# ginevracoal/robustBNNs

Measured on AMD Instinct MI355X. Metric: attack-samples/sec (test_pts x posterior_samples x PGD_iters), higher is better.
Workload: dtype f32 (full-width operands as three f16 pieces: 6 exact f16 MFMA product terms per fp32 product, f32 accumulate)

## Files before the change

robustbnns_amd/csrc/rbnn_triple.hip:

```cpp
#include "rbnn_pieces.hpp"
#include <algorithm>
#include <cstdlib>

namespace {

#ifndef RBNN_X3_PAIR_NOP
#define RBNN_X3_PAIR_NOP 0
#endif
#if RBNN_X3_PAIR_NOP
#define RBNN_X3_PAIR_PAD "\n\ts_nop 1"
#else
#define RBNN_X3_PAIR_PAD ""
#endif
#define RBNN_X3_PAIR_BODY \
    "v_bfe_i32 %[me], %[mw], %[b0], 1\n\t" \
    "v_bfe_i32 %[mo], %[mw], %[b1], 1\n\t" \
    "v_bfi_b32 %[me], %[me], %[cp], %[cn]\n\t" \
    "v_bfi_b32 %[mo], %[mo], %[cp], %[cn]\n\t" \
    "v_fma_mixlo_f16 %[d0], %[ge], %[me], 0\n\t" \
    "v_fma_mixhi_f16 %[d0], %[go], %[mo], 0\n\t" \
    "v_fma_mix_f32 %[re], %[ge], %[me], -%[d0] op_sel_hi:[0,0,1]\n\t" \
    "v_fma_mix_f32 %[ro], %[go], %[mo], -%[d0] op_sel:[0,0,1] op_sel_hi:[0,0,1]\n\t" \
    "v_cvt_pk_f16_f32 %[d1], %[re], %[ro]\n\t" \
    "v_fma_mixlo_f16 %[d2], -%[d1], %[one], %[re] op_sel_hi:[1,0,0]\n\t" \
    "v_fma_mixhi_f16 %[d2], -%[d1], %[one], %[ro] op_sel:[1,0,0] op_sel_hi:[1,0,0]" RBNN_X3_PAIR_PAD
#define RBNN_X3_PAIR_OPS \
    : [d0] "=&v"(d0), [d1] "=&v"(d1), [d2] "=&v"(d2), [me] "=&v"(me), [mo] "=&v"(mo), [re] "=&v"(re), [ro] "=&v"(ro) \
    : [ge] "v"(ge), [go] "v"(go), [mw] "v"(mw), [cp] "v"(cp), [cn] "v"(cn), [one] "v"(one), [b0] "n"(BIT), [b1] "n"(BIT + 1)
template <int BIT, bool FIRST>
__device__ __forceinline__ void split3_pair(float ge, float go, unsigned mw, unsigned cp, unsigned cn, float one,
                                            unsigned& d0, unsigned& d1, unsigned& d2) {
    unsigned me, mo;
    float re, ro;
    if constexpr (FIRST) asm volatile("s_nop 7\n\t" RBNN_X3_PAIR_BODY RBNN_X3_PAIR_OPS);
    else asm volatile(RBNN_X3_PAIR_BODY RBNN_X3_PAIR_OPS);
}

template <bool FIRST>
__device__ __forceinline__ void split3_pair_m(float ge, float go, float me, float mo, float one, unsigned& d0, unsigned& d1, unsigned& d2) {
    float re, ro;
#define RBNN_X3_PAIRM_BODY \
    "v_fma_mixlo_f16 %[d0], %[ge], %[me], 0\n\t" \
    "v_fma_mixhi_f16 %[d0], %[go], %[mo], 0\n\t" \
    "v_fma_mix_f32 %[re], %[ge], %[me], -%[d0] op_sel_hi:[0,0,1]\n\t" \
    "v_fma_mix_f32 %[ro], %[go], %[mo], -%[d0] op_sel:[0,0,1] op_sel_hi:[0,0,1]\n\t" \
    "v_cvt_pk_f16_f32 %[d1], %[re], %[ro]\n\t" \
    "v_fma_mixlo_f16 %[d2], -%[d1], %[one], %[re] op_sel_hi:[1,0,0]\n\t" \
    "v_fma_mixhi_f16 %[d2], -%[d1], %[one], %[ro] op_sel:[1,0,0] op_sel_hi:[1,0,0]" RBNN_X3_PAIR_PAD
#define RBNN_X3_PAIRM_OPS \
    : [d0] "=&v"(d0), [d1] "=&v"(d1), [d2] "=&v"(d2), [re] "=&v"(re), [ro] "=&v"(ro) \
    : [ge] "v"(ge), [go] "v"(go), [me] "v"(me), [mo] "v"(mo), [one] "v"(one)
    if constexpr (FIRST) asm volatile("s_nop 7\n\t" RBNN_X3_PAIRM_BODY RBNN_X3_PAIRM_OPS);
    else asm volatile(RBNN_X3_PAIRM_BODY RBNN_X3_PAIRM_OPS);
}


__global__ void triple_rows_kernel(const float* __restrict__ src, long long rows, int cols, int ld_src, float scale,
                                   const rbnn_dev_scale* __restrict__ ds, uint4* __restrict__ dst, int groups, int grouped) {
    const long long i = (long long)blockIdx.x * blockDim.x + threadIdx.x;
    if (i >= rows * groups) return;
    if (ds) scale = ds->scale;
    const long long r = i / groups;
    const int g = (int)(i % groups);
    const float* const p = src + r * ld_src + 8 * g;
    union { f16x8 v; uint4 u; } o[3];
#pragma unroll
    for (int j = 0; j < 8; ++j) {
        const float v = (8 * g + j < cols) ? p[j] * scale : 0.f;
        _Float16 q[3];
        pieces_of<3>(v, q);
        o[0].v[j] = q[0]; o[1].v[j] = q[1]; o[2].v[j] = q[2];
    }
    if (grouped) {
        uint4* const out = dst + (((r >> 4) * (groups >> 2) + (g >> 2)) * 192 + (r & 15) * 4 + (g & 3));
        out[0] = o[0].u; out[64] = o[1].u; out[128] = o[2].u;
        return;
    }
    uint4* const out = dst + (r * (groups >> 2) + (g >> 2)) * 12 + (g & 3);
    out[0] = o[0].u; out[4] = o[1].u; out[8] = o[2].u;
}

struct FwdX3Args {
    const char* X;  int ldx;  int N;
    const char* W;  long long w_sample_bytes;  int ldw;  int KT;
    const float* b;  const float* W2;  const float* b2;  int C;  int H;
    const int* sidx;  int S;  int NT;  float out_scale;
    float* P;  uint32_t* mask;  float* dact;  int out_kind;
    const rbnn_dev_scale* x_ds;
    long long x_sample_bytes;  char* hid;  float hid_scale;  const rbnn_dev_scale* hid_ds;
    unsigned x_group_bytes, x_stage_bytes;
};

template <int ACT, int WH, int HTW, int WN, int NTW, bool LAYER2, bool XF32 = false>
__global__ void __launch_bounds__(64 * WH * WN, WH * WN / 4) fc_forward_x3_kernel(const FwdX3Args a) {
    constexpr int BH = WH * HTW * 16, BN = WN * NTW * 16;
    constexpr int PLANEB = (BH + BN) * 64;
    constexpr int TILEB = 3 * PLANEB;
    constexpr bool BITMASK = (ACT == RBNN_ACT_RELU || ACT == RBNN_ACT_LEAKY);
    constexpr int NW = WH * WN;
    constexpr int WPP = BH / 16 / NW, XPP = BN / 16 / NW;
    static_assert((BH / 16) % NW == 0 && (BN / 16) % NW == 0, "whole pieces per wave");
    static_assert(HTW % 2 == 0 && HTW <= 8, "a wave's h range is whole 32-bit mask words, at most 4");
    static_assert(WH * BN * 64 <= 2 * TILEB, "the Z^T reduction scratch aliases the tile buffers");
    extern __shared__ __attribute__((aligned(16))) float lds[];
    char* const ldsb = (char*)lds;
    float* const zred = lds;

    int id;
    if (!item_of_block(blockIdx.x, a.NT * a.S, id)) return;
    constexpr int SB = 4;
    int ntile, s;
    {
        const int full = a.S / SB, per = SB * a.NT;
        if (id < full * per) { ntile = (id % per) / SB; s = (id / per) * SB + id % SB; }
        else { const int rem = id - full * per, cnt = a.S - full * SB; ntile = rem / cnt; s = full * SB + rem % cnt; }
    }
    const int tid = threadIdx.x, lane = tid & 63, li = lane & 15, lg = lane >> 4;
    const int wave = __builtin_amdgcn_readfirstlane(tid >> 6);
    const int wave_h = wave % WH, wave_n = wave / WH;
    const int sw = a.sidx ? a.sidx[s] : s;
    const float out_scale = a.x_ds ? a.out_scale * a.x_ds->inv_scale : a.out_scale;
    const float hid_scale = (!LAYER2 && a.hid_ds) ? a.hid_ds->scale : a.hid_scale;
    const char* const Ws = a.W + (long long)sw * a.w_sample_bytes;
    const char* const Xs = a.X + (long long)s * a.x_sample_bytes;
    const int n0 = ntile * BN;
    const int HW = a.H >> 5;
    const int prow = lane >> 2;
    const unsigned src_off = (unsigned)(prow * 64 + ((lane & 3) ^ swz(prow)) * 16);
    const int foff = li * 64 + ((lg ^ swz(li)) * 16);
    auto sw8 = [](int r) { return ((r >> 1) & 1) | (((r >> 2) & 1) << 2); };
    const unsigned src_off_f = (unsigned)((lane >> 3) * 128 + (((lane & 7) ^ sw8(lane >> 3)) * 16));
    const int foff_f0 = li * 128 + (((2 * lg) ^ sw8(li)) * 16), foff_f1 = li * 128 + (((2 * lg + 1) ^ sw8(li)) * 16);

    f32x4 zacc[NTW];
#pragma unroll
    for (int nt = 0; nt < NTW; ++nt) zacc[nt] = (f32x4){0.f, 0.f, 0.f, 0.f};
    if (NW == 8 && wave >= 4) __builtin_amdgcn_s_setprio(1);

    unsigned xrow[XPP], wrow[WPP];
#pragma unroll
    for (int i = 0; i < XPP; ++i) xrow[i] = (unsigned)min((n0 >> 4) + wave + NW * i, ((a.N + 15) >> 4) - 1) * a.x_group_bytes + (XF32 ? src_off_f : src_off);
#pragma unroll
    for (int i = 0; i < WPP; ++i) wrow[i] = (unsigned)(wave + NW * i) * (unsigned)a.KT * 3072u + src_off;

    constexpr int PPS = WPP + XPP;
    const int G = (a.H / BH) * a.KT;
    auto piece = [&](int c, int kt, int buf, int j) {
        char* const T = ldsb + buf * TILEB;
        const char* src;
        char* dst;
        if (j < WPP) {
            src = Ws + (long long)c * BH * a.ldw * 6 + (wrow[j < WPP ? j : 0] + (unsigned)kt * 3072u);
            dst = T + (wave + NW * j) * 3072;
        } else {
            src = Xs + (xrow[j >= WPP ? j - WPP : 0] + (unsigned)kt * a.x_stage_bytes);
            dst = T + (BH / 16 + wave + NW * (j - WPP)) * 3072;
        }
        const auto gsrc = (const __attribute__((address_space(1))) void*)src;
        const auto ldst = (__attribute__((address_space(3))) void*)(uintptr_t)(uint32_t)(uintptr_t)dst;
        __builtin_amdgcn_global_load_lds(gsrc, ldst, 16, 0, 0);
        __builtin_amdgcn_global_load_lds(gsrc, ldst, 16, 1024, 0);
        if (!(XF32 && j >= WPP)) __builtin_amdgcn_global_load_lds(gsrc, ldst, 16, 2048, 0);
    };
#pragma unroll
    for (int i = 0; i < PPS; ++i) piece(0, 0, 0, i);
    ring_wait_barrier<0>();

    f32x4 acc[HTW][NTW];
#pragma unroll
    for (int ht = 0; ht < HTW; ++ht)
#pragma unroll
        for (int nt = 0; nt < NTW; ++nt) acc[ht][nt] = (f32x4){0.f, 0.f, 0.f, 0.f};

    int kt = 0, ch = 0;
    for (int g = 0; g < G; ++g) {
        const int buf = g & 1;
        const bool wrap = kt + 1 == a.KT, last = g + 1 == G;
        const int ktn = last ? kt : (wrap ? 0 : kt + 1), chn = (wrap && !last) ? ch + 1 : ch;
        const char* const Wt = ldsb + buf * TILEB + (wave_h * HTW) * 3072 + foff;
        const char* const Xt = ldsb + buf * TILEB + (BH / 16 + wave_n * NTW) * 3072 + foff;
        f16x8 b0[NTW], b1[NTW], b2[NTW], a0, a1, a2, a0n, a1n, a2n;
        if (!(RBNN_ABL & 1)) {
#pragma unroll
            for (int i = 0; i < PPS; ++i) piece(chn, ktn, buf ^ 1, i);
        }
        if constexpr (XF32) {
            const char* const Xf = ldsb + buf * TILEB + (BH / 16 + wave_n * NTW) * 3072;
            f32x4 x0[NTW], x1[NTW];
#pragma unroll
            for (int nt = 0; nt < NTW; ++nt) {
                x0[nt] = *(const f32x4*)(Xf + nt * 3072 + foff_f0);
                x1[nt] = *(const f32x4*)(Xf + nt * 3072 + foff_f1);
            }
#pragma unroll
            for (int nt = 0; nt < NTW; ++nt) {
                union { f16x8 v; unsigned w[4]; } q0, q1, q2;
                split3_plain_pair(x0[nt][0], x0[nt][1], 1.f, q0.w[0], q1.w[0], q2.w[0]);
                split3_plain_pair(x0[nt][2], x0[nt][3], 1.f, q0.w[1], q1.w[1], q2.w[1]);
                split3_plain_pair(x1[nt][0], x1[nt][1], 1.f, q0.w[2], q1.w[2], q2.w[2]);
                split3_plain_pair(x1[nt][2], x1[nt][3], 1.f, q0.w[3], q1.w[3], q2.w[3]);
                b0[nt] = q0.v; b1[nt] = q1.v; b2[nt] = q2.v;
            }
        } else {
#pragma unroll
            for (int nt = 0; nt < NTW; ++nt) {
                b0[nt] = *(const f16x8*)(Xt + nt * 3072);
                b1[nt] = *(const f16x8*)(Xt + nt * 3072 + 1024);
                b2[nt] = *(const f16x8*)(Xt + nt * 3072 + 2048);
            }
        }
        a0 = *(const f16x8*)(Wt);
        a1 = *(const f16x8*)(Wt + 1024);
        a2 = *(const f16x8*)(Wt + 2048);
        a0n = a0; a1n = a1; a2n = a2;
#pragma unroll
        for (int ht = 0; ht < HTW; ++ht) {
#pragma unroll
            for (int k = 0; k < 6; ++k) {
                const f16x8 av = (k == 1) ? a2 : ((k == 2 || k == 3) ? a1 : a0);
#pragma unroll
                for (int nt = 0; nt < NTW; ++nt) {
                    const f16x8 bv = (k == 0) ? b2[nt] : ((k == 2 || k == 4) ? b1[nt] : b0[nt]);
                    acc[ht][nt] = MFMA_H(av, bv, acc[ht][nt]);
                }
                if (k == 0 && ht + 1 < HTW) {
                    a0n = *(const f16x8*)(Wt + (ht + 1) * 3072);
                    a1n = *(const f16x8*)(Wt + (ht + 1) * 3072 + 1024);
                    a2n = *(const f16x8*)(Wt + (ht + 1) * 3072 + 2048);
                }
            }
            a0 = a0n; a1 = a1n; a2 = a2n;
        }
        {
            __builtin_amdgcn_sched_group_barrier(0x100, 3 * NTW + 3, 0);
#pragma unroll
            for (int ht = 0; ht < HTW; ++ht) {
                __builtin_amdgcn_sched_group_barrier(0x008, 3 * NTW, 0);
                if (ht + 1 < HTW) __builtin_amdgcn_sched_group_barrier(0x100, 3, 0);
                __builtin_amdgcn_sched_group_barrier(0x008, 3 * NTW, 0);
            }
        }
        if (!(RBNN_ABL & 2)) ring_wait_barrier<0>();
        const int hc0 = ch * BH;
        kt = wrap ? 0 : kt + 1;
        ch = wrap ? ch + 1 : ch;
        if (!wrap) continue;

        if (RBNN_ABL & 8) {
            float t = 0.f;
#pragma unroll
            for (int ht = 0; ht < HTW; ++ht)
#pragma unroll
                for (int nt = 0; nt < NTW; ++nt) { t += acc[ht][nt][0] + acc[ht][nt][1] + acc[ht][nt][2] + acc[ht][nt][3]; acc[ht][nt] = (f32x4){0.f, 0.f, 0.f, 0.f}; }
            if (t == 12345.678f) a.P[tid] = t;
            continue;
        }
        const int hw0 = hc0 + (wave_h * HTW) * 16;
        unsigned mine[NTW];
#pragma unroll
        for (int nt = 0; nt < NTW; ++nt) mine[nt] = 0u;
#pragma unroll
        for (int ht = 0; ht < HTW; ++ht) {
            const int hrow = hw0 + ht * 16 + 4 * lg;
            const f32x4 bias = *(const f32x4*)(a.b + (long long)sw * a.H + hrow);
            f32x4 w2f = (f32x4){0.f, 0.f, 0.f, 0.f};
            if (LAYER2 && li < a.C) w2f = *(const f32x4*)(a.W2 + ((long long)sw * a.C + li) * a.H + hrow);
#pragma unroll
            for (int nt = 0; nt < NTW; ++nt) {
                const int n = n0 + (wave_n * NTW + nt) * 16 + li;
                f32x4 v = acc[ht][nt] * out_scale + bias, hv;
                acc[ht][nt] = (f32x4){0.f, 0.f, 0.f, 0.f};
                unsigned bits = 0;
#pragma unroll
                for (int r = 0; r < 4; ++r) {
                    bits |= (v[r] > 0.f ? 1u : 0u) << r;
                    hv[r] = act_fwd<ACT>(v[r]);
                }
                if (BITMASK) {
                    unsigned part = bits << (16 * (ht & 1) + 4 * lg);
                    part |= __shfl_xor(part, 16);
                    part |= __shfl_xor(part, 32);
                    if (lg == (ht >> 1)) mine[nt] |= part;
                }
                if (!BITMASK && a.dact && n < a.N) {
                    f32x4 dv;
#pragma unroll
                    for (int r = 0; r < 4; ++r) dv[r] = act_grad_from_value<ACT>(hv[r]);
                    *(f32x4*)(a.dact + ((long long)s * a.N + n) * a.H + hrow) = dv;
                }
                if (LAYER2) {
#pragma unroll
                    for (int r = 0; r < 4; ++r) zacc[nt] = MFMA16(w2f[r], hv[r], zacc[nt]);
                } else {
#ifdef RBNN_X3_L1_ABL_NOSTORE
                    if (n < a.N && hv[0] == 1.2345e-30f) {
#else
                    if (n < a.N) {
#endif
                        const long long blk = ((long long)s * HW + (hrow >> 5)) * ((a.N + 15) >> 4) + (n >> 4);
#ifdef RBNN_X3_L1_ABL_SMALL
                        char* const row = a.hid + ((blk * 2048) & 0xFFC00) + (n & 15) * 128 + ((hrow >> 4) & 1) * 64 + lg * 16;
#else
                        char* const row = a.hid + blk * 2048 + (n & 15) * 128 + ((hrow >> 4) & 1) * 64 + lg * 16;
#endif
                        *(f32x4*)row = hv * hid_scale;
                    }
                }
            }
        }
        if (BITMASK && a.mask) {
#pragma unroll
            for (int nt = 0; nt < NTW; ++nt) {
                const int n = n0 + (wave_n * NTW + nt) * 16 + li;
                if (lg < HTW / 2 && n < a.N) a.mask[((long long)s * HW + (hw0 >> 5) + lg) * mask_ld(a.N) + n] = mine[nt];
            }
        }
    }
    if (RBNN_ABL & 2) ring_wait_barrier<0>();

    if (!LAYER2) return;
#pragma unroll
    for (int nt = 0; nt < NTW; ++nt)
        *(f32x4*)(zred + (wave_h * BN + (wave_n * NTW + nt) * 16 + li) * 16 + 4 * lg) = zacc[nt];
    __syncthreads();
    if (tid < BN) {
        const int n = n0 + tid;
        float z[16];
#pragma unroll
        for (int q = 0; q < 4; ++q) {
            f32x4 sum = *(const f32x4*)(zred + tid * 16 + 4 * q);
#pragma unroll
            for (int w = 1; w < WH; ++w) sum += *(const f32x4*)(zred + (w * BN + tid) * 16 + 4 * q);
#pragma unroll
            for (int r = 0; r < 4; ++r) z[4 * q + r] = sum[r];
        }
        float m = -INFINITY;
#pragma unroll
        for (int c = 0; c < 16; ++c) {
            if (c < a.C) { z[c] += a.b2[(long long)sw * a.C + c]; m = fmaxf(m, z[c]); }
            else z[c] = 0.f;
        }
        if (a.out_kind == RBNN_OUT_PROBS) {
            float den = 0.f;
#pragma unroll
            for (int c = 0; c < 16; ++c) if (c < a.C) { z[c] = expf(z[c] - m); den += z[c]; }
#pragma unroll
            for (int c = 0; c < 16; ++c) if (c < a.C) z[c] = z[c] / den;
        }
        if (n < a.N) {
            float* const dst = a.P + ((long long)s * a.N + n) * RBNN_CPAD;
#pragma unroll
            for (int q = 0; q < 4; ++q) *(f32x4*)(dst + 4 * q) = (f32x4){z[4 * q], z[4 * q + 1], z[4 * q + 2], z[4 * q + 3]};
        }
    }
}

template <int ACT, int WH, int HTW, int WN, int NTW, bool LAYER2, bool XF32>
int launch_forward_x3_cfg(FwdX3Args a, hipStream_t st) {
    constexpr int BH = WH * HTW * 16, BN = WN * NTW * 16;
    constexpr int LDSB = 2 * 3 * (BH + BN) * 64;
    static_assert(LDSB <= 160 * 1024, "LDS");
    a.NT = (a.N + BN - 1) / BN;
    auto kern = fc_forward_x3_kernel<ACT, WH, HTW, WN, NTW, LAYER2, XF32>;
    static unsigned long long attr_done = 0;
    if (!ensure_dynamic_lds((const void*)kern, LDSB, attr_done)) return RBNN_ERR_LAUNCH;
    const int grid = grid_for_items((long long)a.NT * a.S);
    hipLaunchKernelGGL(kern, dim3(grid), dim3(64 * WH * WN), LDSB, st, a);
    return launch_status();
}

template <int ACT, bool LAYER2, bool XF32>
int launch_forward_x3_act(const FwdX3Args& a, hipStream_t st) {
    if (a.H % 256 == 0) return launch_forward_x3_cfg<ACT, 4, 4, 2, 4, LAYER2, XF32>(a, st);
    if (a.H % 128 == 0) return launch_forward_x3_cfg<ACT, 2, 4, 2, 4, LAYER2, XF32>(a, st);
    return RBNN_ERR_UNSUPPORTED;
}

template <bool LAYER2, bool XF32 = false>
int launch_forward_x3(int act, const FwdX3Args& a, hipStream_t st) {
    return for_activation(act, [&](auto A) { return launch_forward_x3_act<decltype(A)::value, LAYER2, XF32>(a, st); });
}

__global__ void triple_cols_kernel(const float* __restrict__ W, long long n_mats, int rows, int cols, int ld_src, float scale,
                                   uint4* __restrict__ dst, int ld_dst) {
    const long long i = (long long)blockIdx.x * blockDim.x + threadIdx.x;
    const int HB = rows / 32;
    if (i >= n_mats * HB * 4 * ld_dst) return;
    const int d = (int)(i % ld_dst);
    const int lg = (int)((i / ld_dst) % 4);
    const long long mh = i / (4LL * ld_dst);
    const long long m = mh / HB;
    const int hb = (int)(mh % HB);
    union { f16x8 v; uint4 u; } o[3];
#pragma unroll
    for (int j = 0; j < 8; ++j) {
        const int h = 32 * hb + 16 * (j >> 2) + 4 * lg + (j & 3);
        const float v = (d < cols) ? W[(m * rows + h) * ld_src + d] * scale : 0.f;
        _Float16 q[3];
        pieces_of<3>(v, q);
        o[0].v[j] = q[0]; o[1].v[j] = q[1]; o[2].v[j] = q[2];
    }
    const long long base = ((mh * 4 + lg) * 3) * ld_dst;
    dst[base + d] = o[0].u;
    dst[base + ld_dst + d] = o[1].u;
    dst[base + 2 * ld_dst + d] = o[2].u;
}

__global__ void triple_w2gen_kernel(const float* __restrict__ W2, int n_mats, int C, int H, float scale, uint4* __restrict__ dst) {
    const long long i = (long long)blockIdx.x * blockDim.x + threadIdx.x;
    if (i >= (long long)n_mats * (H / 16) * 128) return;
    const int lane = (int)(i & 63), li = lane & 15, lg = lane >> 4, k = (int)((i >> 6) & 1);
    const int t = (int)((i >> 7) % (H / 16));
    const long long m = (i >> 7) / (H / 16);
    _Float16 w[10][3];
#pragma unroll
    for (int c = 0; c < 10; ++c) pieces_of<3>((c < C) ? W2[(m * C + c) * H + 16 * t + li] * scale : 0.f, w[c]);
    union { f16x8 v; uint4 u; } o;
    const _Float16 z = (_Float16)0.f;
    if (lg < 3) {
        const int piece = (k == 0) ? (lg == 2 ? 1 : 0) : (lg == 0 ? 1 : (lg == 1 ? 0 : 2));
#pragma unroll
        for (int j = 0; j < 8; ++j) o.v[j] = piece == 0 ? w[j][0] : (piece == 1 ? w[j][1] : w[j][2]);
    } else if (k == 0) {
        o.v[0] = w[8][0]; o.v[1] = w[9][0]; o.v[2] = w[8][0]; o.v[3] = w[9][0];
        o.v[4] = w[8][0]; o.v[5] = w[9][0]; o.v[6] = w[8][1]; o.v[7] = w[9][1];
    } else {
        o.v[0] = w[8][2]; o.v[1] = w[9][2]; o.v[2] = w[8][1]; o.v[3] = w[9][1];
        o.v[4] = z; o.v[5] = z; o.v[6] = z; o.v[7] = z;
    }
    dst[i] = o.u;
}

__host__ __device__ __forceinline__ int dz_swz3(long long n) { return (int)((0 - (n >> 2)) & 3); }

__global__ void __launch_bounds__(256) triple_dz_kernel(const float* __restrict__ dZ, int S, int N, long long N_pad, int C,
                                                        uint4* __restrict__ dst, float* __restrict__ gscale) {
    __shared__ float red[16][17];
    const int p = threadIdx.x & 15, q = threadIdx.x >> 4;
    const long long n = (long long)blockIdx.x * 16 + p;
    float m = 0.f;
    if (n < N)
        for (int s = q; s < S; s += 16) {
            const float* const src = dZ + ((long long)s * N + n) * RBNN_CPAD;
#pragma unroll
            for (int k = 0; k < 3; ++k) {
                const f32x4 v = *(const f32x4*)(src + 4 * k);
#pragma unroll
                for (int r = 0; r < 4; ++r) if (4 * k + r < C) m = fmaxf(m, fabsf(v[r]));
            }
        }
    red[q][p] = m;
    __syncthreads();
    m = 0.f;
#pragma unroll
    for (int i = 0; i < 16; ++i) m = fmaxf(m, red[i][p]);
    int e = 0;
    if (m > 0.f && m < INFINITY) e = min(13 - ilogbf(m), 120);
    if (q == 0) gscale[n] = ldexpf(1.f, -e);
    const int sw = dz_swz3(n);
    for (int s = q; s < S; s += 16) {
        _Float16 d[10][3];
        float v[12];
        if (n < N) {
            const float* const src = dZ + ((long long)s * N + n) * RBNN_CPAD;
#pragma unroll
            for (int k = 0; k < 3; ++k) {
                const f32x4 t = *(const f32x4*)(src + 4 * k);
#pragma unroll
                for (int r = 0; r < 4; ++r) v[4 * k + r] = t[r];
            }
        }
#pragma unroll
        for (int c = 0; c < 10; ++c) pieces_of<3>((n < N && c < C) ? ldexpf(v[c], e) : 0.f, d[c]);
        uint4* const o = dst + ((long long)s * N_pad + n) * 4;
#pragma unroll
        for (int ch = 0; ch < 3; ++ch) {
            union { f16x8 v; uint4 u; } w;
#pragma unroll
            for (int j = 0; j < 8; ++j) w.v[j] = d[j][ch];
            o[ch ^ sw] = w.u;
        }
        union { f16x8 v; uint4 u; } t;
        t.v[0] = d[8][0]; t.v[1] = d[9][0]; t.v[2] = d[8][1]; t.v[3] = d[9][1];
        t.v[4] = d[8][2]; t.v[5] = d[9][2]; t.v[6] = d[8][0]; t.v[7] = d[9][0];
        o[3 ^ sw] = t.u;
    }
}

template <int MODE>
__device__ __forceinline__ void tail_dz(const float* __restrict__ prow, const float (&gmean)[16], int y, int C, float inv_S, float (&out)[16]) {
    float p[16], g[16];
#pragma unroll
    for (int q = 0; q < 4; ++q) {
        const f32x4 v = *(const f32x4*)(prow + 4 * q);
#pragma unroll
        for (int r = 0; r < 4; ++r) p[4 * q + r] = v[r];
    }
    if (MODE == RBNN_LOSS_PER_SAMPLE) {
        ce_softmax_grad<16>(p, C, y, inv_S, g);
    } else {
#pragma unroll
        for (int c = 0; c < 16; ++c) g[c] = gmean[c];
    }
    if (MODE == RBNN_LOSS_MEAN_LOGIT) {
#pragma unroll
        for (int c = 0; c < 16; ++c) out[c] = g[c];
    } else {
        softmax_backward<16>(g, p, C, out);
    }
}

template <int MODE>
__global__ void __launch_bounds__(256) step_tail_x3_kernel(const float* __restrict__ P, const int* __restrict__ labels, int S, float inv_S, int N,
                                                           long long N_pad, int C, float* __restrict__ Psum_out, int ldo,
                                                           uint4* __restrict__ dst, float* __restrict__ gscale) {
    __shared__ float red[16][17];
    __shared__ float psum[16][16];
    const int p = threadIdx.x & 15, q = threadIdx.x >> 4;
    const long long n = (long long)blockIdx.x * 16 + p;
    if (MODE != RBNN_LOSS_PER_SAMPLE) {
        if (q < 4) {
            f32x4 sum = (f32x4){0.f, 0.f, 0.f, 0.f};
            if (n < N)
                for (int s = 0; s < S; ++s) sum += *(const f32x4*)(P + ((long long)s * N + n) * RBNN_CPAD + 4 * q);
#pragma unroll
            for (int r = 0; r < 4; ++r) {
                psum[p][4 * q + r] = sum[r];
                if (Psum_out && n < N && 4 * q + r < C) Psum_out[n * ldo + 4 * q + r] = sum[r];
            }
        }
        __syncthreads();
    }
    const int y = (n < N) ? labels[n] : 0;
    float gmean[16];
    if (MODE != RBNN_LOSS_PER_SAMPLE) {
        float t[16];
#pragma unroll
        for (int c = 0; c < 16; ++c) t[c] = (c < C) ? psum[p][c] * inv_S : 0.f;
        ce_softmax_grad<16>(t, C, y, inv_S, gmean);
    } else {
#pragma unroll
        for (int c = 0; c < 16; ++c) gmean[c] = 0.f;
    }
    float m = 0.f;
    if (n < N)
        for (int s = q; s < S; s += 16) {
            float dz[16];
            tail_dz<MODE>(P + ((long long)s * N + n) * RBNN_CPAD, gmean, y, C, inv_S, dz);
#pragma unroll
            for (int c = 0; c < 12; ++c) if (c < C) m = fmaxf(m, fabsf(dz[c]));
        }
    red[q][p] = m;
    __syncthreads();
    m = 0.f;
#pragma unroll
    for (int i = 0; i < 16; ++i) m = fmaxf(m, red[i][p]);
    int e = 0;
    if (m > 0.f && m < INFINITY) e = min(13 - ilogbf(m), 120);
    if (q == 0) gscale[n] = ldexpf(1.f, -e);
    const int sw = dz_swz3(n);
    for (int s = q; s < S; s += 16) {
        _Float16 d[10][3];
        float dz[16];
#pragma unroll
        for (int c = 0; c < 16; ++c) dz[c] = 0.f;
        if (n < N) tail_dz<MODE>(P + ((long long)s * N + n) * RBNN_CPAD, gmean, y, C, inv_S, dz);
#pragma unroll
        for (int c = 0; c < 10; ++c) pieces_of<3>((n < N && c < C) ? ldexpf(dz[c], e) : 0.f, d[c]);
        uint4* const o = dst + ((long long)s * N_pad + n) * 4;
#pragma unroll
        for (int ch = 0; ch < 3; ++ch) {
            union { f16x8 v; uint4 u; } w;
#pragma unroll
            for (int j = 0; j < 8; ++j) w.v[j] = d[j][ch];
            o[ch ^ sw] = w.u;
        }
        union { f16x8 v; uint4 u; } t;
        t.v[0] = d[8][0]; t.v[1] = d[9][0]; t.v[2] = d[8][1]; t.v[3] = d[9][1];
        t.v[4] = d[8][2]; t.v[5] = d[9][2]; t.v[6] = d[8][0]; t.v[7] = d[9][0];
        o[3 ^ sw] = t.u;
    }
}

__global__ void __launch_bounds__(256) attack_step_x3_kernel(float* __restrict__ X, const float* __restrict__ X0, int ldx, const float* __restrict__ G,
                                                             int K, long long slab_stride, int ldg, const float* __restrict__ alpha, float alpha_scalar,
                                                             float eps, int project, long long N, int D, const rbnn_dev_scale* __restrict__ ds,
                                                             uint4* __restrict__ dst, int groups) {
    const long long i = (long long)blockIdx.x * blockDim.x + threadIdx.x;
    if (i >= N * groups) return;
    const long long n = i / groups;
    const int gq = (int)(i % groups), d0 = 8 * gq;
    const float scale = ds->scale;
    float xn[8];
#pragma unroll
    for (int j = 0; j < 8; ++j) xn[j] = 0.f;
    if (d0 < D) {
        const float step = alpha ? alpha[n] : alpha_scalar;
#pragma unroll
        for (int h = 0; h < 2; ++h) {
            const int d = d0 + 4 * h;
            if (d < D) {
                f32x4 g = *(const f32x4*)(G + n * ldg + d);
                for (int k = 1; k < K; ++k) g += *(const f32x4*)(G + k * slab_stride + n * ldg + d);
                const f32x4 x = *(const f32x4*)(X + n * ldx + d);
                f32x4 x0 = x, out;
                if (project) x0 = *(const f32x4*)(X0 + n * ldx + d);
#pragma unroll
                for (int r = 0; r < 4; ++r) {
                    const float sgn = (g[r] > 0.f) ? 1.f : ((g[r] < 0.f) ? -1.f : 0.f);
                    float pert = x[r] + step * sgn;
                    if (project) pert = x0[r] + fminf(fmaxf(pert - x0[r], -eps), eps);
                    out[r] = fminf(fmaxf(pert, 0.f), 1.f);
                    xn[4 * h + r] = out[r];
                }
                *(f32x4*)(X + n * ldx + d) = out;
            }
        }
    }
    union { f16x8 v; uint4 u; } o[3];
#pragma unroll
    for (int j = 0; j < 8; ++j) {
        _Float16 q[3];
        pieces_of<3>((d0 + j < D) ? xn[j] * scale : 0.f, q);
        o[0].v[j] = q[0]; o[1].v[j] = q[1]; o[2].v[j] = q[2];
    }
    uint4* const out = dst + (((n >> 4) * (groups >> 2) + (gq >> 2)) * 192 + (n & 15) * 4 + (gq & 3));
    out[0] = o[0].u; out[64] = o[1].u; out[128] = o[2].u;
}

template <int ACT, int TD, int MODE>
__global__ void __launch_bounds__(256, 2) fc_grad_x3_kernel(const GradPieceArgs a) {
    constexpr int NW = 4;
    constexpr bool GEN = MODE != GRAD_FC2_STEP2;
    constexpr bool BITMASK = (ACT == RBNN_ACT_RELU || ACT == RBNN_ACT_LEAKY);
    constexpr bool STREAM = !GEN || !BITMASK;
    constexpr int NTW = 16 / NW, BM = 256, LD = TD * 16;
    constexpr int W1B = 12 * LD * 16;
    constexpr int NPIECE = W1B / 1024, PPW = (NPIECE + NW - 1) / NW;
    constexpr int BUFB = W1B + 4096 + 1024;
    constexpr int DZB = BM * 64;
    static_assert(W1B % 1024 == 0, "whole DMA pieces");
    extern __shared__ __attribute__((aligned(16))) float lds[];
    char* const ldsb = (char*)lds;
    char* const dzl = ldsb + 2 * BUFB;

    int id;
    if (!item_of_block(blockIdx.x, a.NT * a.ND * a.nchunks, id)) return;
    int ntile, dg, ch;
    grad_item(id, a.NT, a.ND, STREAM, ntile, dg, ch);
    const int tid = threadIdx.x, lane = tid & 63, li = lane & 15, lg = lane >> 4;
    const int wave = __builtin_amdgcn_readfirstlane(tid >> 6);
    const int nb = ntile * BM + wave * (NTW * 16);
    const int dc0 = dg * LD;
    const int Dp = a.Dt * 16;
    const int ntd = min(TD, a.Dt - dg * TD);
    const int s_begin = ch * a.chunk, s_end = min(a.S, s_begin + a.chunk);
    const int HS = a.H / 32, nst = (s_end - s_begin) * HS;

    unsigned goff[PPW];
#pragma unroll
    for (int i = 0; i < PPW; ++i) {
        const int f = (wave + NW * i) * 1024 + lane * 16, seg = f / (LD * 16), d = (f % (LD * 16)) >> 4;
        goff[i] = (unsigned)(seg * a.ldc + min(dc0 + d, a.ldc - 1)) * 16u;
    }
    const unsigned loff = (unsigned)lane * 16u;

    f32x4 acc[NTW][TD];
#pragma unroll
    for (int nt = 0; nt < NTW; ++nt)
#pragma unroll
        for (int dt = 0; dt < TD; ++dt) acc[nt][dt] = (f32x4){0.f, 0.f, 0.f, 0.f};

    auto dz_issue = [&](int s) {
        const char* const src = a.dzg + ((long long)s * a.n_pad + nb) * 64;
#pragma unroll
// ... 338 lines not shown
```

Baseline: 139.6 million.

## Process two hidden chunks per X tile load in forward x3 kernel

Adds an NCH=2 path, used by default when H is a multiple of 512. Each X k-tile is loaded and split once and reused against two consecutive W hidden chunks held in a W ring, with two accumulator sets. This halves the X global-to-LDS traffic and the XF32 splitting work per hidden chunk. In exchange it doubles accumulator registers, which may lower occupancy or cause spills, and it adds an extra barrier per k-step. The epilogue is moved into a shared include file.

New measurement: 144.8 million (median of 6 runs). 3.7% higher.

```diff
diff --git a/robustbnns_amd/csrc/rbnn_triple.hip b/robustbnns_amd/csrc/rbnn_triple.hip
--- a/robustbnns_amd/csrc/rbnn_triple.hip
+++ b/robustbnns_amd/csrc/rbnn_triple.hip
@@ -91,7 +91,7 @@
     unsigned x_group_bytes, x_stage_bytes;
 };
 
-template <int ACT, int WH, int HTW, int WN, int NTW, bool LAYER2, bool XF32 = false>
+template <int ACT, int WH, int HTW, int WN, int NTW, bool LAYER2, bool XF32 = false, int NCH = 1>
 __global__ void __launch_bounds__(64 * WH * WN, WH * WN / 4) fc_forward_x3_kernel(const FwdX3Args a) {
     constexpr int BH = WH * HTW * 16, BN = WN * NTW * 16;
     constexpr int PLANEB = (BH + BN) * 64;
@@ -143,177 +143,242 @@
 #pragma unroll
     for (int i = 0; i < WPP; ++i) wrow[i] = (unsigned)(wave + NW * i) * (unsigned)a.KT * 3072u + src_off;
 
-    constexpr int PPS = WPP + XPP;
-    const int G = (a.H / BH) * a.KT;
-    auto piece = [&](int c, int kt, int buf, int j) {
-        char* const T = ldsb + buf * TILEB;
-        const char* src;
-        char* dst;
-        if (j < WPP) {
-            src = Ws + (long long)c * BH * a.ldw * 6 + (wrow[j < WPP ? j : 0] + (unsigned)kt * 3072u);
-            dst = T + (wave + NW * j) * 3072;
-        } else {
-            src = Xs + (xrow[j >= WPP ? j - WPP : 0] + (unsigned)kt * a.x_stage_bytes);
-            dst = T + (BH / 16 + wave + NW * (j - WPP)) * 3072;
-        }
-        const auto gsrc = (const __attribute__((address_space(1))) void*)src;
-        const auto ldst = (__attribute__((address_space(3))) void*)(uintptr_t)(uint32_t)(uintptr_t)dst;
-        __builtin_amdgcn_global_load_lds(gsrc, ldst, 16, 0, 0);
-        __builtin_amdgcn_global_load_lds(gsrc, ldst, 16, 1024, 0);
-        if (!(XF32 && j >= WPP)) __builtin_amdgcn_global_load_lds(gsrc, ldst, 16, 2048, 0);
+    auto abl_keep_live = [&](f32x4 (&acc)[HTW][NTW]) {
+        float t = 0.f;
+#pragma unroll
+        for (int ht = 0; ht < HTW; ++ht)
+#pragma unroll
+            for (int nt = 0; nt < NTW; ++nt) { t += acc[ht][nt][0] + acc[ht][nt][1] + acc[ht][nt][2] + acc[ht][nt][3]; acc[ht][nt] = (f32x4){0.f, 0.f, 0.f, 0.f}; }
+        if (t == 12345.678f) a.P[tid] = t;
     };
-#pragma unroll
-    for (int i = 0; i < PPS; ++i) piece(0, 0, 0, i);
-    ring_wait_barrier<0>();
-
-    f32x4 acc[HTW][NTW];
-#pragma unroll
-    for (int ht = 0; ht < HTW; ++ht)
-#pragma unroll
-        for (int nt = 0; nt < NTW; ++nt) acc[ht][nt] = (f32x4){0.f, 0.f, 0.f, 0.f};
-
-    int kt = 0, ch = 0;
-    for (int g = 0; g < G; ++g) {
-        const int buf = g & 1;
-        const bool wrap = kt + 1 == a.KT, last = g + 1 == G;
-        const int ktn = last ? kt : (wrap ? 0 : kt + 1), chn = (wrap && !last) ? ch + 1 : ch;
-        const char* const Wt = ldsb + buf * TILEB + (wave_h * HTW) * 3072 + foff;
-        const char* const Xt = ldsb + buf * TILEB + (BH / 16 + wave_n * NTW) * 3072 + foff;
-        f16x8 b0[NTW], b1[NTW], b2[NTW], a0, a1, a2, a0n, a1n, a2n;
-        if (!(RBNN_ABL & 1)) {
-#pragma unroll
-            for (int i = 0; i < PPS; ++i) piece(chn, ktn, buf ^ 1, i);
-        }
-        if constexpr (XF32) {
-            const char* const Xf = ldsb + buf * TILEB + (BH / 16 + wave_n * NTW) * 3072;
-            f32x4 x0[NTW], x1[NTW];
-#pragma unroll
-            for (int nt = 0; nt < NTW; ++nt) {
-                x0[nt] = *(const f32x4*)(Xf + nt * 3072 + foff_f0);
-                x1[nt] = *(const f32x4*)(Xf + nt * 3072 + foff_f1);
-            }
-#pragma unroll
-            for (int nt = 0; nt < NTW; ++nt) {
-                union { f16x8 v; unsigned w[4]; } q0, q1, q2;
-                split3_plain_pair(x0[nt][0], x0[nt][1], 1.f, q0.w[0], q1.w[0], q2.w[0]);
-                split3_plain_pair(x0[nt][2], x0[nt][3], 1.f, q0.w[1], q1.w[1], q2.w[1]);
-                split3_plain_pair(x1[nt][0], x1[nt][1], 1.f, q0.w[2], q1.w[2], q2.w[2]);
-                split3_plain_pair(x1[nt][2], x1[nt][3], 1.f, q0.w[3], q1.w[3], q2.w[3]);
-                b0[nt] = q0.v; b1[nt] = q1.v; b2[nt] = q2.v;
-            }
-        } else {
-#pragma unroll
-            for (int nt = 0; nt < NTW; ++nt) {
-                b0[nt] = *(const f16x8*)(Xt + nt * 3072);
-                b1[nt] = *(const f16x8*)(Xt + nt * 3072 + 1024);
-                b2[nt] = *(const f16x8*)(Xt + nt * 3072 + 2048);
-            }
-        }
-        a0 = *(const f16x8*)(Wt);
-        a1 = *(const f16x8*)(Wt + 1024);
-        a2 = *(const f16x8*)(Wt + 2048);
-        a0n = a0; a1n = a1; a2n = a2;
-#pragma unroll
-        for (int ht = 0; ht < HTW; ++ht) {
-#pragma unroll
-            for (int k = 0; k < 6; ++k) {
-                const f16x8 av = (k == 1) ? a2 : ((k == 2 || k == 3) ? a1 : a0);
-#pragma unroll
-                for (int nt = 0; nt < NTW; ++nt) {
-                    const f16x8 bv = (k == 0) ? b2[nt] : ((k == 2 || k == 4) ? b1[nt] : b0[nt]);
-                    acc[ht][nt] = MFMA_H(av, bv, acc[ht][nt]);
-                }
-                if (k == 0 && ht + 1 < HTW) {
-                    a0n = *(const f16x8*)(Wt + (ht + 1) * 3072);
-                    a1n = *(const f16x8*)(Wt + (ht + 1) * 3072 + 1024);
-                    a2n = *(const f16x8*)(Wt + (ht + 1) * 3072 + 2048);
-                }
-            }
-            a0 = a0n; a1 = a1n; a2 = a2n;
-        }
-        {
-            __builtin_amdgcn_sched_group_barrier(0x100, 3 * NTW + 3, 0);
+
+    if constexpr (NCH == 2) {
+        constexpr int WBUFB = BH / 16 * 3072, XBUFB = BN / 16 * 3072;
+        static_assert(2 * (WBUFB + XBUFB) == 2 * TILEB, "same LDS");
+        char* const Wring = ldsb;
+        char* const Xring = ldsb + 2 * WBUFB;
+        auto dma = [&](const char* src, char* dst, bool third) {
+            const auto gsrc = (const __attribute__((address_space(1))) void*)src;
+            const auto ldst = (__attribute__((address_space(3))) void*)(uintptr_t)(uint32_t)(uintptr_t)dst;
+            __builtin_amdgcn_global_load_lds(gsrc, ldst, 16, 0, 0);
+            __builtin_amdgcn_global_load_lds(gsrc, ldst, 16, 1024, 0);
+            if (third) __builtin_amdgcn_global_load_lds(gsrc, ldst, 16, 2048, 0);
+        };
+        auto w_groups = [&](int c, int kt, int buf) {
+#pragma unroll
+            for (int j = 0; j < WPP; ++j)
+                dma(Ws + (long long)c * BH * a.ldw * 6 + (wrow[j] + (unsigned)kt * 3072u), Wring + buf * WBUFB + (wave + NW * j) * 3072, true);
+        };
+        auto x_groups = [&](int kt, int buf) {
+#pragma unroll
+            for (int j = 0; j < XPP; ++j)
+                dma(Xs + (xrow[j] + (unsigned)kt * a.x_stage_bytes), Xring + buf * XBUFB + (wave + NW * j) * 3072, !XF32);
+        };
+        auto mma = [&](f32x4 (&accc)[HTW][NTW], const char* const Wt, const f16x8 (&b0)[NTW], const f16x8 (&b1)[NTW],
+                       const f16x8 (&b2)[NTW]) __attribute__((always_inline)) {
+            f16x8 a0 = *(const f16x8*)(Wt), a1 = *(const f16x8*)(Wt + 1024), a2 = *(const f16x8*)(Wt + 2048), a0n = a0, a1n = a1, a2n = a2;
+#pragma unroll
+            for (int ht = 0; ht < HTW; ++ht) {
+#pragma unroll
+                for (int k = 0; k < 6; ++k) {
+                    const f16x8 av = (k == 1) ? a2 : ((k == 2 || k == 3) ? a1 : a0);
+#pragma unroll
+                    for (int nt = 0; nt < NTW; ++nt) {
+                        const f16x8 bv = (k == 0) ? b2[nt] : ((k == 2 || k == 4) ? b1[nt] : b0[nt]);
+                        accc[ht][nt] = MFMA_H(av, bv, accc[ht][nt]);
+                    }
+                    if (k == 0 && ht + 1 < HTW) {
+                        a0n = *(const f16x8*)(Wt + (ht + 1) * 3072);
+                        a1n = *(const f16x8*)(Wt + (ht + 1) * 3072 + 1024);
+                        a2n = *(const f16x8*)(Wt + (ht + 1) * 3072 + 2048);
+                    }
+                }
+                a0 = a0n; a1 = a1n; a2 = a2n;
+            }
+        };
+        auto pin = [&](auto lead) __attribute__((always_inline)) {
+            __builtin_amdgcn_sched_group_barrier(0x100, decltype(lead)::value, 0);
 #pragma unroll
             for (int ht = 0; ht < HTW; ++ht) {
                 __builtin_amdgcn_sched_group_barrier(0x008, 3 * NTW, 0);
                 if (ht + 1 < HTW) __builtin_amdgcn_sched_group_barrier(0x100, 3, 0);
                 __builtin_amdgcn_sched_group_barrier(0x008, 3 * NTW, 0);
             }
-        }
-        if (!(RBNN_ABL & 2)) ring_wait_barrier<0>();
-        const int hc0 = ch * BH;
-        kt = wrap ? 0 : kt + 1;
-        ch = wrap ? ch + 1 : ch;
-        if (!wrap) continue;
-
-        if (RBNN_ABL & 8) {
-            float t = 0.f;
+        };
+        auto epilogue = [&](f32x4 (&acc)[HTW][NTW], const int hc0) {
+            if (RBNN_ABL & 8) { abl_keep_live(acc); return; }
+#include "rbnn_triple_fwd_epilogue.inc"
+        };
+        w_groups(0, 0, 0);
+        x_groups(0, 0);
+        ring_wait_barrier<0>();
+
+        f32x4 acc[2][HTW][NTW];
+#pragma unroll
+        for (int c = 0; c < 2; ++c)
 #pragma unroll
             for (int ht = 0; ht < HTW; ++ht)
 #pragma unroll
-                for (int nt = 0; nt < NTW; ++nt) { t += acc[ht][nt][0] + acc[ht][nt][1] + acc[ht][nt][2] + acc[ht][nt][3]; acc[ht][nt] = (f32x4){0.f, 0.f, 0.f, 0.f}; }
-            if (t == 12345.678f) a.P[tid] = t;
-            continue;
-        }
-        const int hw0 = hc0 + (wave_h * HTW) * 16;
-        unsigned mine[NTW];
-#pragma unroll
-        for (int nt = 0; nt < NTW; ++nt) mine[nt] = 0u;
-#pragma unroll
-        for (int ht = 0; ht < HTW; ++ht) {
-            const int hrow = hw0 + ht * 16 + 4 * lg;
-            const f32x4 bias = *(const f32x4*)(a.b + (long long)sw * a.H + hrow);
-            f32x4 w2f = (f32x4){0.f, 0.f, 0.f, 0.f};
-            if (LAYER2 && li < a.C) w2f = *(const f32x4*)(a.W2 + ((long long)sw * a.C + li) * a.H + hrow);
-#pragma unroll
-            for (int nt = 0; nt < NTW; ++nt) {
-                const int n = n0 + (wave_n * NTW + nt) * 16 + li;
-                f32x4 v = acc[ht][nt] * out_scale + bias, hv;
-                acc[ht][nt] = (f32x4){0.f, 0.f, 0.f, 0.f};
-                unsigned bits = 0;
-#pragma unroll
-                for (int r = 0; r < 4; ++r) {
-                    bits |= (v[r] > 0.f ? 1u : 0u) << r;
-                    hv[r] = act_fwd<ACT>(v[r]);
-                }
-                if (BITMASK) {
-                    unsigned part = bits << (16 * (ht & 1) + 4 * lg);
-                    part |= __shfl_xor(part, 16);
-                    part |= __shfl_xor(part, 32);
-                    if (lg == (ht >> 1)) mine[nt] |= part;
-                }
-                if (!BITMASK && a.dact && n < a.N) {
-                    f32x4 dv;
-#pragma unroll
-                    for (int r = 0; r < 4; ++r) dv[r] = act_grad_from_value<ACT>(hv[r]);
-                    *(f32x4*)(a.dact + ((long long)s * a.N + n) * a.H + hrow) = dv;
-                }
-                if (LAYER2) {
-#pragma unroll
-                    for (int r = 0; r < 4; ++r) zacc[nt] = MFMA16(w2f[r], hv[r], zacc[nt]);
-                } else {
-#ifdef RBNN_X3_L1_ABL_NOSTORE
-                    if (n < a.N && hv[0] == 1.2345e-30f) {
-#else
-                    if (n < a.N) {
-#endif
-                        const long long blk = ((long long)s * HW + (hrow >> 5)) * ((a.N + 15) >> 4) + (n >> 4);
-#ifdef RBNN_X3_L1_ABL_SMALL
-                        char* const row = a.hid + ((blk * 2048) & 0xFFC00) + (n & 15) * 128 + ((hrow >> 4) & 1) * 64 + lg * 16;
-#else
-                        char* const row = a.hid + blk * 2048 + (n & 15) * 128 + ((hrow >> 4) & 1) * 64 + lg * 16;
-#endif
-                        *(f32x4*)row = hv * hid_scale;
+                for (int nt = 0; nt < NTW; ++nt) acc[c][ht][nt] = (f32x4){0.f, 0.f, 0.f, 0.f};
+
+        const int T = (a.H / (2 * BH)) * a.KT;
+        int kt = 0, pr = 0, xb = 0;
+        for (int t = 0; t < T; ++t) {
+            const bool wrap = kt + 1 == a.KT, last = t + 1 == T;
+            const int ktn = last ? kt : (wrap ? 0 : kt + 1), cn = last ? 2 * pr + 1 : (wrap ? 2 * pr + 2 : 2 * pr);
+            const char* const Wt = Wring + (wave_h * HTW) * 3072 + foff;
+            const char* const Xt = Xring + xb * XBUFB + (wave_n * NTW) * 3072;
+            f16x8 b0[NTW], b1[NTW], b2[NTW];
+            if (!(RBNN_ABL & 1)) w_groups(2 * pr + 1, kt, 1);
+            if constexpr (XF32) {
+                f32x4 x0[NTW], x1[NTW];
+#pragma unroll
+                for (int nt = 0; nt < NTW; ++nt) {
+                    x0[nt] = *(const f32x4*)(Xt + nt * 3072 + foff_f0);
+                    x1[nt] = *(const f32x4*)(Xt + nt * 3072 + foff_f1);
+                }
+#pragma unroll
+                for (int nt = 0; nt < NTW; ++nt) {
+                    union { f16x8 v; unsigned w[4]; } q0, q1, q2;
+                    split3_plain_pair(x0[nt][0], x0[nt][1], 1.f, q0.w[0], q1.w[0], q2.w[0]);
+                    split3_plain_pair(x0[nt][2], x0[nt][3], 1.f, q0.w[1], q1.w[1], q2.w[1]);
+                    split3_plain_pair(x1[nt][0], x1[nt][1], 1.f, q0.w[2], q1.w[2], q2.w[2]);
+                    split3_plain_pair(x1[nt][2], x1[nt][3], 1.f, q0.w[3], q1.w[3], q2.w[3]);
+                    b0[nt] = q0.v; b1[nt] = q1.v; b2[nt] = q2.v;
+                }
+            } else {
+#pragma unroll
+                for (int nt = 0; nt < NTW; ++nt) {
+                    b0[nt] = *(const f16x8*)(Xt + foff + nt * 3072);
+                    b1[nt] = *(const f16x8*)(Xt + foff + nt * 3072 + 1024);
+                    b2[nt] = *(const f16x8*)(Xt + foff + nt * 3072 + 2048);
+                }
+            }
+            mma(acc[0], Wt, b0, b1, b2);
+            pin(std::integral_constant<int, 3 * NTW + 3>());
+            if (!(RBNN_ABL & 2)) ring_wait_barrier<0>();
+            __builtin_amdgcn_sched_barrier(0);
+            if (!(RBNN_ABL & 1)) {
+                w_groups(cn, ktn, 0);
+                x_groups(ktn, xb ^ 1);
+            }
+            mma(acc[1], Wt + WBUFB, b0, b1, b2);
+            pin(std::integral_constant<int, 3>());
+            if (!(RBNN_ABL & 2)) ring_wait_barrier<0>();
+            xb ^= 1;
+            const int hc0 = 2 * pr * BH;
+            kt = wrap ? 0 : kt + 1;
+            pr = wrap ? pr + 1 : pr;
+            if (wrap) {
+#pragma unroll
+                for (int c = 0; c < 2; ++c) epilogue(acc[c], hc0 + c * BH);
+            }
+        }
+    } else {
+        constexpr int PPS = WPP + XPP;
+        const int G = (a.H / BH) * a.KT;
+        auto piece = [&](int c, int kt, int buf, int j) {
+            char* const T = ldsb + buf * TILEB;
+            const char* src;
+            char* dst;
+            if (j < WPP) {
+                src = Ws + (long long)c * BH * a.ldw * 6 + (wrow[j < WPP ? j : 0] + (unsigned)kt * 3072u);
+                dst = T + (wave + NW * j) * 3072;
+            } else {
+                src = Xs + (xrow[j >= WPP ? j - WPP : 0] + (unsigned)kt * a.x_stage_bytes);
+                dst = T + (BH / 16 + wave + NW * (j - WPP)) * 3072;
+            }
+            const auto gsrc = (const __attribute__((address_space(1))) void*)src;
+            const auto ldst = (__attribute__((address_space(3))) void*)(uintptr_t)(uint32_t)(uintptr_t)dst;
+            __builtin_amdgcn_global_load_lds(gsrc, ldst, 16, 0, 0);
+            __builtin_amdgcn_global_load_lds(gsrc, ldst, 16, 1024, 0);
+            if (!(XF32 && j >= WPP)) __builtin_amdgcn_global_load_lds(gsrc, ldst, 16, 2048, 0);
+        };
+#pragma unroll
+        for (int i = 0; i < PPS; ++i) piece(0, 0, 0, i);
+        ring_wait_barrier<0>();
+
+        f32x4 acc[HTW][NTW];
+#pragma unroll
+        for (int ht = 0; ht < HTW; ++ht)
+#pragma unroll
+            for (int nt = 0; nt < NTW; ++nt) acc[ht][nt] = (f32x4){0.f, 0.f, 0.f, 0.f};
+
+        int kt = 0, ch = 0;
+        for (int g = 0; g < G; ++g) {
+            const int buf = g & 1;
+            const bool wrap = kt + 1 == a.KT, last = g + 1 == G;
+            const int ktn = last ? kt : (wrap ? 0 : kt + 1), chn = (wrap && !last) ? ch + 1 : ch;
+            const char* const Wt = ldsb + buf * TILEB + (wave_h * HTW) * 3072 + foff;
+            const char* const Xt = ldsb + buf * TILEB + (BH / 16 + wave_n * NTW) * 3072 + foff;
+            f16x8 b0[NTW], b1[NTW], b2[NTW], a0, a1, a2, a0n, a1n, a2n;
+            if (!(RBNN_ABL & 1)) {
+#pragma unroll
+                for (int i = 0; i < PPS; ++i) piece(chn, ktn, buf ^ 1, i);
+            }
+            if constexpr (XF32) {
+                const char* const Xf = ldsb + buf * TILEB + (BH / 16 + wave_n * NTW) * 3072;
+                f32x4 x0[NTW], x1[NTW];
+#pragma unroll
+                for (int nt = 0; nt < NTW; ++nt) {
+                    x0[nt] = *(const f32x4*)(Xf + nt * 3072 + foff_f0);
+                    x1[nt] = *(const f32x4*)(Xf + nt * 3072 + foff_f1);
+                }
+#pragma unroll
+                for (int nt = 0; nt < NTW; ++nt) {
+                    union { f16x8 v; unsigned w[4]; } q0, q1, q2;
+                    split3_plain_pair(x0[nt][0], x0[nt][1], 1.f, q0.w[0], q1.w[0], q2.w[0]);
+                    split3_plain_pair(x0[nt][2], x0[nt][3], 1.f, q0.w[1], q1.w[1], q2.w[1]);
+                    split3_plain_pair(x1[nt][0], x1[nt][1], 1.f, q0.w[2], q1.w[2], q2.w[2]);
+                    split3_plain_pair(x1[nt][2], x1[nt][3], 1.f, q0.w[3], q1.w[3], q2.w[3]);
+                    b0[nt] = q0.v; b1[nt] = q1.v; b2[nt] = q2.v;
+                }
+            } else {
+#pragma unroll
+                for (int nt = 0; nt < NTW; ++nt) {
+                    b0[nt] = *(const f16x8*)(Xt + nt * 3072);
+                    b1[nt] = *(const f16x8*)(Xt + nt * 3072 + 1024);
+                    b2[nt] = *(const f16x8*)(Xt + nt * 3072 + 2048);
+                }
+            }
+            a0 = *(const f16x8*)(Wt);
+            a1 = *(const f16x8*)(Wt + 1024);
+            a2 = *(const f16x8*)(Wt + 2048);
+            a0n = a0; a1n = a1; a2n = a2;
+#pragma unroll
+            for (int ht = 0; ht < HTW; ++ht) {
+#pragma unroll
+                for (int k = 0; k < 6; ++k) {
+                    const f16x8 av = (k == 1) ? a2 : ((k == 2 || k == 3) ? a1 : a0);
+#pragma unroll
+                    for (int nt = 0; nt < NTW; ++nt) {
+                        const f16x8 bv = (k == 0) ? b2[nt] : ((k == 2 || k == 4) ? b1[nt] : b0[nt]);
+                        acc[ht][nt] = MFMA_H(av, bv, acc[ht][nt]);
                     }
-                }
-            }
-        }
-        if (BITMASK && a.mask) {
-#pragma unroll
-            for (int nt = 0; nt < NTW; ++nt) {
-                const int n = n0 + (wave_n * NTW + nt) * 16 + li;
-                if (lg < HTW / 2 && n < a.N) a.mask[((long long)s * HW + (hw0 >> 5) + lg) * mask_ld(a.N) + n] = mine[nt];
-            }
+                    if (k == 0 && ht + 1 < HTW) {
+                        a0n = *(const f16x8*)(Wt + (ht + 1) * 3072);
+                        a1n = *(const f16x8*)(Wt + (ht + 1) * 3072 + 1024);
+                        a2n = *(const f16x8*)(Wt + (ht + 1) * 3072 + 2048);
+                    }
+                }
+                a0 = a0n; a1 = a1n; a2 = a2n;
+            }
+            {
+                __builtin_amdgcn_sched_group_barrier(0x100, 3 * NTW + 3, 0);
+#pragma unroll
+                for (int ht = 0; ht < HTW; ++ht) {
+                    __builtin_amdgcn_sched_group_barrier(0x008, 3 * NTW, 0);
+                    if (ht + 1 < HTW) __builtin_amdgcn_sched_group_barrier(0x100, 3, 0);
+                    __builtin_amdgcn_sched_group_barrier(0x008, 3 * NTW, 0);
+                }
+            }
+            if (!(RBNN_ABL & 2)) ring_wait_barrier<0>();
+            const int hc0 = ch * BH;
+            kt = wrap ? 0 : kt + 1;
+            ch = wrap ? ch + 1 : ch;
+            if (!wrap) continue;
+            if (RBNN_ABL & 8) { abl_keep_live(acc); continue; }
+#include "rbnn_triple_fwd_epilogue.inc"
         }
     }
     if (RBNN_ABL & 2) ring_wait_barrier<0>();
@@ -355,13 +420,13 @@
     }
 }
 
-template <int ACT, int WH, int HTW, int WN, int NTW, bool LAYER2, bool XF32>
+template <int ACT, int WH, int HTW, int WN, int NTW, bool LAYER2, bool XF32, int NCH = 1>
 int launch_forward_x3_cfg(FwdX3Args a, hipStream_t st) {
     constexpr int BH = WH * HTW * 16, BN = WN * NTW * 16;
     constexpr int LDSB = 2 * 3 * (BH + BN) * 64;
     static_assert(LDSB <= 160 * 1024, "LDS");
     a.NT = (a.N + BN - 1) / BN;
-    auto kern = fc_forward_x3_kernel<ACT, WH, HTW, WN, NTW, LAYER2, XF32>;
+    auto kern = fc_forward_x3_kernel<ACT, WH, HTW, WN, NTW, LAYER2, XF32, NCH>;
     static unsigned long long attr_done = 0;
     if (!ensure_dynamic_lds((const void*)kern, LDSB, attr_done)) return RBNN_ERR_LAUNCH;
     const int grid = grid_for_items((long long)a.NT * a.S);
@@ -371,6 +436,10 @@
 
 template <int ACT, bool LAYER2, bool XF32>
 int launch_forward_x3_act(const FwdX3Args& a, hipStream_t st) {
+    if (a.H % 512 == 0) {
+        const char* const e = getenv("RBNN_X3_FWD_XONCE");
+        if (!e || e[0] != '0') return launch_forward_x3_cfg<ACT, 4, 4, 2, 4, LAYER2, XF32, 2>(a, st);
+    }
     if (a.H % 256 == 0) return launch_forward_x3_cfg<ACT, 4, 4, 2, 4, LAYER2, XF32>(a, st);
     if (a.H % 128 == 0) return launch_forward_x3_cfg<ACT, 2, 4, 2, 4, LAYER2, XF32>(a, st);
     return RBNN_ERR_UNSUPPORTED;
diff --git a/robustbnns_amd/csrc/rbnn_triple_fwd_epilogue.inc b/robustbnns_amd/csrc/rbnn_triple_fwd_epilogue.inc
--- /dev/null
+++ b/robustbnns_amd/csrc/rbnn_triple_fwd_epilogue.inc
@@ -0,0 +1,60 @@
+        const int hw0 = hc0 + (wave_h * HTW) * 16;
+        unsigned mine[NTW];
+#pragma unroll
+        for (int nt = 0; nt < NTW; ++nt) mine[nt] = 0u;
+#pragma unroll
+        for (int ht = 0; ht < HTW; ++ht) {
+            const int hrow = hw0 + ht * 16 + 4 * lg;
+            const f32x4 bias = *(const f32x4*)(a.b + (long long)sw * a.H + hrow);
+            f32x4 w2f = (f32x4){0.f, 0.f, 0.f, 0.f};
+            if (LAYER2 && li < a.C) w2f = *(const f32x4*)(a.W2 + ((long long)sw * a.C + li) * a.H + hrow);
+#pragma unroll
+            for (int nt = 0; nt < NTW; ++nt) {
+                const int n = n0 + (wave_n * NTW + nt) * 16 + li;
+                f32x4 v = acc[ht][nt] * out_scale + bias, hv;
+                acc[ht][nt] = (f32x4){0.f, 0.f, 0.f, 0.f};
+                unsigned bits = 0;
+#pragma unroll
+                for (int r = 0; r < 4; ++r) {
+                    bits |= (v[r] > 0.f ? 1u : 0u) << r;
+                    hv[r] = act_fwd<ACT>(v[r]);
+                }
+                if (BITMASK) {
+                    unsigned part = bits << (16 * (ht & 1) + 4 * lg);
+                    part |= __shfl_xor(part, 16);
+                    part |= __shfl_xor(part, 32);
+                    if (lg == (ht >> 1)) mine[nt] |= part;
+                }
+                if (!BITMASK && a.dact && n < a.N) {
+                    f32x4 dv;
+#pragma unroll
+                    for (int r = 0; r < 4; ++r) dv[r] = act_grad_from_value<ACT>(hv[r]);
+                    *(f32x4*)(a.dact + ((long long)s * a.N + n) * a.H + hrow) = dv;
+                }
+                if (LAYER2) {
+#pragma unroll
+                    for (int r = 0; r < 4; ++r) zacc[nt] = MFMA16(w2f[r], hv[r], zacc[nt]);
+                } else {
+#ifdef RBNN_X3_L1_ABL_NOSTORE
+                    if (n < a.N && hv[0] == 1.2345e-30f) {
+#else
+                    if (n < a.N) {
+#endif
+                        const long long blk = ((long long)s * HW + (hrow >> 5)) * ((a.N + 15) >> 4) + (n >> 4);
+#ifdef RBNN_X3_L1_ABL_SMALL
+                        char* const row = a.hid + ((blk * 2048) & 0xFFC00) + (n & 15) * 128 + ((hrow >> 4) & 1) * 64 + lg * 16;
+#else
+                        char* const row = a.hid + blk * 2048 + (n & 15) * 128 + ((hrow >> 4) & 1) * 64 + lg * 16;
+#endif
+                        *(f32x4*)row = hv * hid_scale;
+                    }
+                }
+            }
+        }
+        if (BITMASK && a.mask) {
+#pragma unroll
+            for (int nt = 0; nt < NTW; ++nt) {
+                const int n = n0 + (wave_n * NTW + nt) * 16 + li;
+                if (lg < HTW / 2 && n < a.N) a.mask[((long long)s * HW + (hw0 >> 5) + lg) * mask_ld(a.N) + n] = mine[nt];
+            }
+        }
```
